# HKUST-Aerial-Robotics/MIND

Hardware: AMD Instinct MI355X
Metric: sim steps/sec (whole node) + scenario-tree nodes expanded/sec, AV2 demo scenes (higher is better)
Workload: dtype f32-class (bf16 hi+mid+lo split operands = 24 significand bits, six products, fp32 accumulate) pair kernel + ActorNet, f32 elsewhere in the predictor, f64 iLQR

## Files before the change

include/mind_hip.h:

```cpp
#ifndef MIND_HIP_H
#define MIND_HIP_H

#include <stddef.h>
#include <stdint.h>

#ifdef __cplusplus
extern "C" {
#endif

#define MIND_OK 0
#define MIND_EINVAL (-1)
#define MIND_ENOMEM (-2)
#define MIND_EHIP (-3)
#define MIND_ESTATE (-4)
#define MIND_ENOTFOUND (-5)

typedef struct mind_ctx mind_ctx;

int mind_ctx_create(int device, void *stream, mind_ctx **out);
int mind_ctx_destroy(mind_ctx *ctx);
const char *mind_last_error_string(mind_ctx *ctx);
int mind_ctx_synchronize(mind_ctx *ctx);

typedef struct {
// ... 44 lines not shown
#define MIND_PAIR_BF16X6 3
int mind_set_pair_precision(mind_ctx *ctx, int mode);

int mind_set_tuning(mind_ctx *ctx, const char *name, int value);
int mind_get_pair_precision(mind_ctx *ctx);
int mind_debug_pack_bfrag(const float *w, int row_stride, uint32_t *out);

int mind_debug_pair_schedule(const int *scene_tokens, const int *scene_actors, int n_scenes, int n_cu, int last_layer, int *out_jobs, int cap,
                             int *out_info);

int mind_debug_actor_lw_plan(int n_actors, int np, int chunk, long long *out_launches, int cap, long long *out_info);

int mind_debug_pack_conv_frag(const float *w, int co, int ci, int ksz, uint32_t *out, size_t cap);

int mind_debug_trig(mind_ctx *ctx, const double *x, int n, double *out);

int mind_debug_set_layers(mind_ctx *ctx, int n);
int64_t mind_debug_read(mind_ctx *ctx, const char *name, float *host, int64_t max_floats);

typedef struct {
  int n_nodes;
  const int32_t *parent;
  const float *prob;
  int n_agents;
  const float *agent_mean;
  const float *agent_cov;
  const double *field;
  const double *node_w;
} mind_cost_tree;

// ... 283 lines not shown
```

mind_amd/_lib.py:

```python
import ctypes as C
import os

_HERE = os.path.dirname(os.path.abspath(__file__))
LIB_PATH = os.environ.get("MIND_HIP_LIB", os.path.join(_HERE, "libmind_hip.so"))

MIND_OK = 0
MIND_EINVAL, MIND_ENOMEM, MIND_EHIP, MIND_ESTATE, MIND_ENOTFOUND = -1, -2, -3, -4, -5


class TensorDesc(C.Structure):
    _fields_ = [("name", C.c_char_p), ("data", C.POINTER(C.c_float)), ("numel", C.c_int64)]


class SceneBatch(C.Structure):
    _fields_ = [("n_scenes", C.c_int), ("actor_off", C.POINTER(C.c_int32)), ("lane_off", C.POINTER(C.c_int32)),
                ("actors", C.c_void_p), ("lanes", C.c_void_p), ("lane_feat", C.c_void_p),
                ("actor_ctrs", C.c_void_p), ("actor_vecs", C.c_void_p), ("lane_ctrs", C.c_void_p),
                ("lane_vecs", C.c_void_p), ("rpe", C.POINTER(C.c_void_p)), ("tgt_nodes", C.c_void_p),
                ("tgt_rpe", C.c_void_p)]


class PredOut(C.Structure):
    _fields_ = [("cls", C.c_void_p), ("reg", C.c_void_p), ("vel", C.c_void_p), ("lane_feat", C.c_void_p),
                ("actor_emb", C.c_void_p), ("cls_emb", C.c_void_p)]
# ... 119 lines not shown
    _fields_ = [("time_ahead", C.c_double), ("min_vel", C.c_float), ("dist_thres", C.c_float), ("max_depth", C.c_int), ("max_rounds", C.c_int),
                ("pred_len", C.c_int), ("prob_floor", C.c_float), ("cfg_warm", C.c_void_p), ("cfg_full", C.c_void_p), ("speculative", C.c_int),
                ("ego_type_slot", C.c_int)]


class PlannerOut(C.Structure):
    _fields_ = [("n_plans", C.c_longlong),
                ("n_agents", C.c_int), ("n_trees", C.c_int), ("best", C.c_int), ("n_expanded", C.c_int), ("n_rounds", C.c_int), ("n_traj_nodes", C.c_int),
                ("costs", C.POINTER(C.c_double)), ("ctrl", C.c_double * 2), ("aime_s", C.c_double), ("ilqr_s", C.c_double), ("total_s", C.c_double),
                ("tot", LoopTotals)]


EXPORTS = ["mind_ctx_create", "mind_ctx_destroy", "mind_last_error_string", "mind_ctx_synchronize",
           "mind_weights_load", "mind_predict_batch", "mind_last_fusion_stats", "mind_last_actor_stats", "mind_debug_actor_lw_plan", "mind_set_profiling",
           "mind_ilqr_solve_trees", "mind_ilqr_contingency", "mind_ilqr_solve_fields", "mind_cost_eval", "mind_lane_dist_field", "mind_aime_world", "mind_aime_rebase", "mind_debug_set_layers",
           "mind_debug_read", "mind_set_pair_precision", "mind_get_pair_precision", "mind_debug_pack_bfrag", "mind_debug_pack_conv_frag", "mind_debug_pair_schedule", "mind_set_tuning", "mind_last_ilqr_stats", "mind_aime_plan", "mind_last_ilqr_profile", "mind_eval_traj_trees", "mind_last_ilqr_trace", "mind_ilqr_contingency_begin", "mind_ilqr_finish", "mind_fill_tracks", "mind_ilqr_contingency_begin_plan", "mind_debug_trig", "mind_aime_plan_begin", "mind_aime_plan_poll", "mind_aime_plan_finish", "mind_ctx_busy", "mind_ilqr_finish_plan",
           "mind_set_exchange", "mind_last_exchange_stats",
           "mind_loop_create", "mind_loop_destroy", "mind_loop_reset", "mind_loop_advance", "mind_loop_state", "mind_loop_last_plan", "mind_loop_export",
           "mind_planner_create", "mind_planner_destroy", "mind_planner_reset", "mind_planner_observe", "mind_planner_set_lanes", "mind_planner_set_target_lane",
           "mind_planner_set_solve_lane", "mind_planner_set_eval_lane", "mind_planner_plan", "mind_planner_last_plan", "mind_planner_export"]

EXCHANGE_FN = C.CFUNCTYPE(C.c_int, C.c_void_p, C.c_int, C.c_void_p, C.c_void_p, C.c_int64)
XCHG_ALLGATHER, XCHG_ALLREDUCE, XCHG_ALLTOALLV = 0, 1, 2

_lib = None


def load():
    global _lib
    if _lib is not None:
        return _lib
# ... 41 lines not shown
    lib.mind_aime_plan_poll.argtypes = [C.c_void_p]
    lib.mind_aime_plan_finish.argtypes = [C.c_void_p, C.POINTER(AimePlanOut)]
    lib.mind_ctx_busy.argtypes = [C.c_void_p]
    lib.mind_ilqr_finish_plan.argtypes = [C.c_void_p, C.c_int, C.c_int, C.c_void_p, C.c_void_p, C.c_void_p, C.c_void_p]
    lib.mind_set_pair_precision.argtypes = [C.c_void_p, C.c_int]
    lib.mind_set_tuning.argtypes = [C.c_void_p, C.c_char_p, C.c_int]
    lib.mind_last_ilqr_stats.argtypes = [C.c_void_p, C.POINTER(C.c_float), C.POINTER(C.c_int), C.POINTER(C.c_int)]
    lib.mind_last_ilqr_profile.argtypes = [C.c_void_p, C.POINTER(C.c_double)]
    lib.mind_last_ilqr_trace.argtypes = [C.c_void_p, C.c_int, C.c_int, C.POINTER(C.c_double), C.c_int, C.POINTER(C.c_int)]
    lib.mind_eval_traj_trees.argtypes = [C.POINTER(C.c_double), C.POINTER(C.c_double), C.POINTER(C.c_int32), C.c_int, C.c_void_p, C.c_int, C.c_int,
                                         C.c_double, C.POINTER(C.c_double)]
    lib.mind_get_pair_precision.argtypes = [C.c_void_p]
    lib.mind_debug_pack_bfrag.argtypes = [C.POINTER(C.c_float), C.c_int, C.POINTER(C.c_uint32)]
    lib.mind_debug_pair_schedule.argtypes = [C.POINTER(C.c_int), C.POINTER(C.c_int), C.c_int, C.c_int, C.c_int, C.POINTER(C.c_int), C.c_int, C.POINTER(C.c_int)]
    lib.mind_debug_trig.argtypes = [C.c_void_p, C.POINTER(C.c_double), C.c_int, C.POINTER(C.c_double)]
    lib.mind_debug_pack_conv_frag.argtypes = [C.POINTER(C.c_float), C.c_int, C.c_int, C.c_int, C.POINTER(C.c_uint32), C.c_size_t]
    lib.mind_debug_set_layers.argtypes = [C.c_void_p, C.c_int]
    lib.mind_debug_read.argtypes = [C.c_void_p, C.c_char_p, C.POINTER(C.c_float), C.c_int64]
    lib.mind_set_exchange.argtypes = [C.c_void_p, C.c_int, C.c_int, EXCHANGE_FN, C.c_void_p, C.c_int]
    lib.mind_last_exchange_stats.argtypes = [C.c_void_p, C.POINTER(C.c_longlong), C.POINTER(C.c_longlong)]
    lib.mind_loop_create.argtypes = [C.c_void_p, C.POINTER(LoopDesc), C.POINTER(C.c_void_p)]
    lib.mind_loop_destroy.argtypes = [C.c_void_p]
    lib.mind_loop_reset.argtypes = [C.c_void_p]
    lib.mind_loop_advance.argtypes = [C.c_void_p, C.c_int, C.c_double, C.c_longlong, C.POINTER(LoopOut)]
    lib.mind_loop_state.argtypes = [C.c_void_p, C.POINTER(LoopOut)]
    lib.mind_loop_last_plan.argtypes = [C.c_void_p, C.POINTER(AimePlanOut)] + [C.POINTER(C.c_void_p)] * 6 + [C.c_void_p]
    lib.mind_loop_export.argtypes = [C.c_void_p, C.c_int, C.POINTER(C.c_int), C.c_void_p, C.c_void_p, C.c_void_p]
    lib.mind_planner_create.argtypes = [C.c_void_p, C.POINTER(PlannerDesc), C.POINTER(C.c_void_p)]
    lib.mind_planner_destroy.argtypes = [C.c_void_p]
    lib.mind_planner_reset.argtypes = [C.c_void_p]
# ... 26 lines not shown
```

mind_amd/csrc/actor_mfma_kernels.hip:

```cpp
#include <hip/hip_runtime.h>
#include <stdint.h>

#define AM_T 1024
#ifdef MIND_ACTOR_TRACE
__device__ long long am_tr_[64];
__device__ int am_trn_;
#define AM_MARK() do { if (blockIdx.x == 0 && threadIdx.x == 0) { const long long n_ = clock64(); am_tr_[am_trn_ & 63] = n_; ++am_trn_; } } while (0)
#else
#define AM_MARK() do {} while (0)
#endif
#define AM_WAVES 16
#define AM_MAXT 2
#define AM_RSD(C) (3 * (C) / 2 + 4)
#define AM_BUF 2496
#define AM_XIN 0
#define AM_O0 1344
#define AM_FA (AM_O0 + 7 * AM_BUF)
#define AM_RED (AM_FA + 48 * AM_RSD(128))
#define AM_LDS_DWORDS (AM_RED + 64)

struct AmRes { const u32 *c1, *c2, *ds; const float *g1, *b1, *g2, *b2, *gd, *bd; };
struct AmLat { const u32 *w; const float *g, *b; };
struct AmW {
  AmRes res[9];
  AmLat lat[4];
};
typedef u32 u32x2 __attribute__((ext_vector_type(2)));

__device__ __forceinline__ float am_block_sum(float v, float *red, int flip) {
  v = wave_sum(v);
  float *r = red + (flip & 1) * 32;
  if ((threadIdx.x & 63) == 0) r[threadIdx.x >> 6] = v;
  __syncthreads();
  float s = 0.f;
#pragma unroll
  for (int w = 0; w < AM_WAVES; ++w) s += r[w];
  return s;
}

template <int NP>
__device__ __forceinline__ void am_store_split(u32 *rowp, int plane, const f32x4 &y) {
  u32x2 h, m, l;
  h[0] = pk_bf16(y[0], y[1]); h[1] = pk_bf16(y[2], y[3]);
  *(u32x2 *)rowp = h;
  if (NP == 1) return;
  const float r0 = y[0] - bf_lo_f32(h[0]), r1 = y[1] - bf_hi_f32(h[0]), r2 = y[2] - bf_lo_f32(h[1]), r3 = y[3] - bf_hi_f32(h[1]);
  m[0] = pk_bf16(r0, r1); m[1] = pk_bf16(r2, r3);
  *(u32x2 *)(rowp + plane) = m;
  l[0] = pk_bf16(r0 - bf_lo_f32(m[0]), r1 - bf_hi_f32(m[0])); l[1] = pk_bf16(r2 - bf_lo_f32(m[1]), r3 - bf_hi_f32(m[1]));
  *(u32x2 *)(rowp + 2 * plane) = l;
}
template <int NP>
// ... 44 lines not shown
      acc[i] = MFMA_BF(ah, bh, acc[i]);
      if (NP >= 3) {
        if (NP == 6) {
          corr = MFMA_BF(al, bh, corr);
          corr = MFMA_BF(ah, bl, corr);
          corr = MFMA_BF(am, bm, corr);
        }
        corr = MFMA_BF(am, bh, corr);
        corr = MFMA_BF(ah, bm, corr);
      }
    }
    if (NP >= 3) acc[i] += corr;
  }
}

template <int NP>
__device__ __forceinline__ void am_gn(f32x4 (&acc)[AM_MAXT], int Cout, int Tout, const float *__restrict__ g,
                                      const float *__restrict__ b, const u32 *resid, const float *up, bool relu, u32 *outs,
                                      float *outf, float *__restrict__ gout, float *red) {
  const int lane = threadIdx.x & 63, wave = threadIdx.x >> 6;
  const int r = lane & 15, q = lane >> 4;
  const int ntt = (Tout + 15) >> 4;
  const int tiles = (Cout >> 4) * ntt;
  const int RSD = AM_RSD(Cout), PLANE = Cout >> 1;
  f32x4 gg[AM_MAXT], bb[AM_MAXT];
  float s = 0.f;
#pragma unroll
  for (int i = 0; i < AM_MAXT; ++i) {
    const int ti = wave + AM_WAVES * i;
    if (ti >= tiles) continue;
    const int mt = ti / ntt, nt = ti - mt * ntt;
    gg[i] = *(const f32x4 *)(g + mt * 16 + q * 4);
    bb[i] = *(const f32x4 *)(b + mt * 16 + q * 4);
    if (nt * 16 + r < Tout) s += (acc[i][0] + acc[i][1]) + (acc[i][2] + acc[i][3]);
  }
  const float n = (float)(Cout * Tout);
  const float mean = am_block_sum(s, red, 0) / n;
  float v = 0.f;
#pragma unroll
  for (int i = 0; i < AM_MAXT; ++i) {
    const int ti = wave + AM_WAVES * i;
    if (ti >= tiles) continue;
    const int nt = ti % ntt;
    if (nt * 16 + r < Tout) {
#pragma unroll
      for (int e = 0; e < 4; ++e) { const float d = acc[i][e] - mean; v = fmaf(d, d, v); }
    }
  }
  const float rstd = 1.0f / sqrtf(am_block_sum(v, red, 1) / n + 1e-5f);
#pragma unroll
  for (int i = 0; i < AM_MAXT; ++i) {
    const int ti = wave + AM_WAVES * i;
    if (ti >= tiles) continue;
    const int mt = ti / ntt, nt = ti - mt * ntt;
    const int t = nt * 16 + r, co = mt * 16 + q * 4;
    if (t >= Tout) continue;
    f32x4 y;
#pragma unroll
    for (int e = 0; e < 4; ++e) y[e] = (acc[i][e] - mean) * rstd * gg[i][e] + bb[i][e];
    if (resid) y += am_load_split<NP>(resid + t * RSD + (co >> 1), PLANE);
    if (up) {
      const int Th = Tout >> 1;
      float sp = (t + 0.5f) * 0.5f - 0.5f;
      sp = sp < 0.f ? 0.f : sp;
// ... 4 lines not shown
#pragma unroll
      for (int e = 0; e < 4; ++e) y[e] += (1.0f - l1) * a0[e] + l1 * a1[e];
    }
    if (relu) {
#pragma unroll
      for (int e = 0; e < 4; ++e) y[e] = fmaxf(y[e], 0.f);
    }
    if (gout) {
      if (t == Tout - 1) *(f32x4 *)(gout + co) = y;
    } else if (outf) {
      *(f32x4 *)(outf + t * 132 + co) = y;
    } else {
      am_store_split<NP>(outs + t * RSD + (co >> 1), PLANE, y);
    }
  }
  __syncthreads();
}

template <int NP, int LGCI, int LGCO, int STRIDE, bool DS>
__device__ __forceinline__ void am_res(const u32 *in, int Tin, const AmRes &W, u32 *out, u32 *t1, u32 *t2, float *red) {
  constexpr int Cout = 1 << LGCO;
  const int Tout = Tin / STRIDE;
  f32x4 acc[AM_MAXT];
  am_conv<NP, LGCI, 3, STRIDE>(in, Tin, W.c1, Cout, Tout, acc);
  AM_MARK();
  am_gn<NP>(acc, Cout, Tout, W.g1, W.b1, nullptr, nullptr, true, t1, nullptr, nullptr, red);
  AM_MARK();
  const u32 *resid = in;
  if (DS) {
    am_conv<NP, LGCI, 1, STRIDE>(in, Tin, W.ds, Cout, Tout, acc);
    AM_MARK();
    am_gn<NP>(acc, Cout, Tout, W.gd, W.bd, nullptr, nullptr, false, t2, nullptr, nullptr, red);
    AM_MARK();
    resid = t2;
  }
  am_conv<NP, LGCO, 3, 1>(t1, Tout, W.c2, Cout, Tout, acc);
  AM_MARK();
  am_gn<NP>(acc, Cout, Tout, W.g2, W.b2, resid, nullptr, true, out, nullptr, nullptr, red);
  AM_MARK();
}

template <int NP, int LGC>
__device__ __forceinline__ void am_lateral(const u32 *src, int T, const AmLat &W, const float *up, float *dstf, u32 *dsts,
                                           float *red) {
  f32x4 acc[AM_MAXT];
  am_conv<NP, LGC, 3, 1>(src, T, W.w, 128, T, acc);
  AM_MARK();
  am_gn<NP>(acc, 128, T, W.g, W.b, nullptr, up, false, dsts, dstf, nullptr, red);
  AM_MARK();
}

template <int NP>
__global__ __launch_bounds__(AM_T) void k_actor_mfma(const float *__restrict__ actors , int n_actors,
                                                     float *__restrict__ out , AmW W) {
  extern __shared__ __attribute__((aligned(16))) u32 smu[];
  u32 *xin = smu + AM_XIN;
  u32 *o0 = smu + AM_O0, *o1 = o0 + AM_BUF, *o2 = o1 + AM_BUF, *o3 = o2 + AM_BUF;
  u32 *ta = o3 + AM_BUF, *tb = ta + AM_BUF, *tc = tb + AM_BUF;
  u32 *fa = smu + AM_FA;
  float *red = (float *)(smu + AM_RED);
  const int tid = threadIdx.x;
  const int a = blockIdx.x;
  if (a >= n_actors) return;
  if (tid < 48 * 8) {
    const int t = tid >> 3, c = (tid & 7) * 2;
    const float v0 = c < 14 ? actors[((size_t)a * 14 + c) * 48 + t] : 0.f;
    const float v1 = c + 1 < 14 ? actors[((size_t)a * 14 + c + 1) * 48 + t] : 0.f;
    u32 *p = xin + t * AM_RSD(16) + (c >> 1);
    const u32 h = pk_bf16(v0, v1);
    const float r0 = v0 - bf_lo_f32(h), r1 = v1 - bf_hi_f32(h);
    const u32 m = pk_bf16(r0, r1);
    p[0] = h; p[8] = m; p[16] = pk_bf16(r0 - bf_lo_f32(m), r1 - bf_hi_f32(m));
  }
  __syncthreads();
#ifdef MIND_ACTOR_TRACE
  if (blockIdx.x == 0 && tid == 0) am_trn_ = 0;
#endif
  AM_MARK();
  am_res<NP, 4, 5, 1, true>(xin, 48, W.res[0], ta, tb, tc, red);
  am_res<NP, 5, 5, 1, false>(ta, 48, W.res[1], o0, tb, tc, red);
  am_res<NP, 5, 6, 2, true>(o0, 48, W.res[2], ta, tb, tc, red);
  am_res<NP, 6, 6, 1, false>(ta, 24, W.res[3], o1, tb, tc, red);
  am_res<NP, 6, 7, 2, true>(o1, 24, W.res[4], ta, tb, tc, red);
  am_res<NP, 7, 7, 1, false>(ta, 12, W.res[5], o2, tb, tc, red);
  am_res<NP, 7, 8, 2, true>(o2, 12, W.res[6], ta, tb, tc, red);
  am_res<NP, 8, 8, 1, false>(ta, 6, W.res[7], o3, tb, tc, red);
  am_lateral<NP, 8>(o3, 6, W.lat[3], nullptr, (float *)ta, nullptr, red);
  am_lateral<NP, 7>(o2, 12, W.lat[2], (const float *)ta, (float *)tb, nullptr, red);
  am_lateral<NP, 6>(o1, 24, W.lat[1], (const float *)tb, (float *)o2, nullptr, red);
  am_lateral<NP, 5>(o0, 48, W.lat[0], (const float *)o2, nullptr, fa, red);
  {
    const AmRes &R = W.res[8];
    f32x4 acc[AM_MAXT];
    am_conv<NP, 7, 3, 1>(fa, 48, R.c1, 128, 48, acc);
    AM_MARK();
    am_gn<NP>(acc, 128, 48, R.g1, R.b1, nullptr, nullptr, true, o0, nullptr, nullptr, red);
    AM_MARK();
    am_conv<NP, 7, 3, 1>(o0, 48, R.c2, 128, 48, acc);
    AM_MARK();
    am_gn<NP>(acc, 128, 48, R.g2, R.b2, fa, nullptr, true, nullptr, nullptr, out + (size_t)a * 128, red);
    AM_MARK();
  }
#ifdef MIND_ACTOR_TRACE
  if (blockIdx.x == 0 && tid == 0) {
    printf("[k_actor_mfma<%d>] cycles conv/gn per stage:", NP);
    for (int q = 1; q < am_trn_ && q < 64; ++q) printf(" %lld", am_tr_[q] - am_tr_[q - 1]);
    printf("\n");
  }
#endif
}
extern "C" size_t mind_actor_mfma_lds_bytes() { return (size_t)AM_LDS_DWORDS * sizeof(u32); }
```

mind_amd/csrc/encdec_kernels.hip:

```cpp
#include <hip/hip_runtime.h>
#include <stdint.h>

typedef float f32x4 __attribute__((ext_vector_type(4)));

#define NT 256

__device__ __forceinline__ float wave_sum(float v) {
  v += __shfl_xor(v, 32, 64);
  v += __shfl_xor(v, 16, 64);
  v += __shfl_xor(v, 8, 64);
  v += __shfl_xor(v, 4, 64);
  v += __shfl_xor(v, 2, 64);
  v += __shfl_xor(v, 1, 64);
  return v;
}

__device__ __forceinline__ float block_sum(float v, float *red) {
  v = wave_sum(v);
  __syncthreads();
  if ((threadIdx.x & 63) == 0) red[threadIdx.x >> 6] = v;
  __syncthreads();
  return red[0] + red[1] + red[2] + red[3];
}

#ifndef DB
#define DB 16
#endif
#define DENSE_ROW_FENCE() __builtin_amdgcn_sched_barrier(0)
#define DBQ 8
template <int R>
__device__ __forceinline__ void dense_quads(const float *in, int ldi, int K, const float *__restrict__ WT,
                                            const float *__restrict__ b, int NOUT, float *out, int ldo,
                                            float *part, int part_floats) {
  const int nthr = blockDim.x;
  const int NQ = NOUT >> 2;
  int KP = 1;
  while (KP * 2 * NQ <= nthr && KP * 2 * R * NOUT <= part_floats && KP * 2 <= (K >> 2)) KP *= 2;
// ... 940 lines not shown
```

mind_amd/csrc/fusion_kernels.hip:

```cpp
#include <hip/hip_runtime.h>
#include <stdint.h>

typedef float f32x4 __attribute__((ext_vector_type(4)));
typedef float f32x16 __attribute__((ext_vector_type(16)));

typedef unsigned int u32;
typedef u32 u32x4 __attribute__((ext_vector_type(4)));
typedef __bf16 bf16x8 __attribute__((ext_vector_type(8)));
typedef __bf16 bf16x2_t __attribute__((ext_vector_type(2)));
typedef float f32x2_t __attribute__((ext_vector_type(2)));

__device__ __forceinline__ u32 pk_bf16(float a, float b) {
  f32x2_t v = {a, b};
  return __builtin_bit_cast(u32, __builtin_convertvector(v, bf16x2_t));
}
__device__ __forceinline__ float bf_lo_f32(u32 pk) { return __builtin_bit_cast(float, pk << 16); }
__device__ __forceinline__ float bf_hi_f32(u32 pk) { return __builtin_bit_cast(float, pk & 0xffff0000u); }

#define D_ 128
#define PART_STRIDE 1040

struct PairJob {
  long long edge_base;
  int N;
// ... 21 lines not shown
#define LDS_WAE 0
#define LDS_WAP 16384
#define LDS_STAGE 32768
#define LDS_PTAB (LDS_STAGE + PAIR_WAVES * STAGE_FLOATS)
#define LDS_SVEC (LDS_PTAB + PAIR_WAVES * 128)
#define LDS_VT (LDS_SVEC + PAIR_WAVES * 136)
#define LDS_RT (LDS_VT + VT_SIZE)
#define LDS_TOTAL (LDS_RT + 1024)

#define LDS_FENCE() asm volatile("s_waitcnt lgkmcnt(0)" ::: "memory")
#define SCHED_FENCE() __builtin_amdgcn_sched_barrier(0)
#define OPAQUE(x) asm volatile("" : "+v"(x))

typedef f32x4 frag8[8];

__device__ __forceinline__ float red_quad(float v) {
  v += __shfl_xor(v, 16, 64);
  v += __shfl_xor(v, 32, 64);
  return v;
}
__device__ __forceinline__ float red_max16(float v) {
  v = fmaxf(v, __shfl_xor(v, 8, 64));
  v = fmaxf(v, __shfl_xor(v, 4, 64));
  v = fmaxf(v, __shfl_xor(v, 2, 64));
  v = fmaxf(v, __shfl_xor(v, 1, 64));
  return v;
}
__device__ __forceinline__ float red_sum16(float v) {
  v += __shfl_xor(v, 8, 64);
  v += __shfl_xor(v, 4, 64);
  v += __shfl_xor(v, 2, 64);
  v += __shfl_xor(v, 1, 64);
  return v;
}

__device__ __forceinline__ void ln_pairs(frag8 &a, const float *vtq, int off_g, int off_b, bool relu) {
  float s = 0.f;
#pragma unroll
  for (int b = 0; b < 8; ++b)
#pragma unroll
    for (int w = 0; w < 4; ++w) s += a[b][w];
  s = red_quad(s);
  const float mean = s * (1.0f / 128.0f);
  float v = 0.f;
#pragma unroll
  for (int b = 0; b < 8; ++b)
#pragma unroll
    for (int w = 0; w < 4; ++w) {
      const float d = a[b][w] - mean;
// ... 459 lines not shown
__device__ __forceinline__ void ksum(const float (&acc)[TP], float bias, float *rk, int kg, int col, float &r0, float &r1) {
  constexpr int TPW = TP;
  __syncthreads();
#pragma unroll
  for (int t = 0; t < TPW; ++t) rk[(kg * TPW + t) * 128 + col] = acc[t];
  __syncthreads();
  const int t0 = (TP / TKG) * kg;
  r0 = ((rk[(0 * TPW + t0) * 128 + col] + rk[(1 * TPW + t0) * 128 + col]) +
        (rk[(2 * TPW + t0) * 128 + col] + rk[(3 * TPW + t0) * 128 + col])) + bias;
  r1 = 0.f;
  if (TP / TKG == 2)
    r1 = ((rk[(0 * TPW + t0 + 1) * 128 + col] + rk[(1 * TPW + t0 + 1) * 128 + col]) +
          (rk[(2 * TPW + t0 + 1) * 128 + col] + rk[(3 * TPW + t0 + 1) * 128 + col])) + bias;
}

__device__ __forceinline__ void gsum2(float &a, float &b, float *rd, int kg, int tid) {
#pragma unroll
  for (int o = 32; o > 0; o >>= 1) { a += __shfl_xor(a, o, 64); b += __shfl_xor(b, o, 64); }
  const int wv = (tid >> 6) & 1;
  __syncthreads();
  if ((tid & 63) == 0) { rd[(kg * 2 + wv) * 2] = a; rd[(kg * 2 + wv) * 2 + 1] = b; }
  __syncthreads();
  a = rd[(kg * 2) * 2] + rd[(kg * 2 + 1) * 2];
  b = rd[(kg * 2) * 2 + 1] + rd[(kg * 2 + 1) * 2 + 1];
}

__device__ __forceinline__ void ln2tok(float &p0, float &p1, float g, float be, float *rd, int kg, int tid) {
  float s0 = p0, s1 = p1;
  gsum2(s0, s1, rd, kg, tid);
  const float d0 = p0 - s0 * (1.0f / 128.0f), d1 = p1 - s1 * (1.0f / 128.0f);
  s0 = d0 * d0; s1 = d1 * d1;
  gsum2(s0, s1, rd, kg, tid);
  p0 = d0 * (1.0f / sqrtf(s0 * (1.0f / 128.0f) + 1e-5f)) * g + be;
  p1 = d1 * (1.0f / sqrtf(s1 * (1.0f / 128.0f) + 1e-5f)) * g + be;
}

template <int TPW, bool MG>
__device__ __forceinline__ void k_token_body(const TokMeta *__restrict__ meta, int n_tok, int mode,
                                             const float *__restrict__ actor_feat,
                                             const float *__restrict__ lane_feat, float *__restrict__ x,
                                             const float *__restrict__ part, float *__restrict__ ST,
                                             float *__restrict__ QK, const TokWeights &W) {
  __shared__ __attribute__((aligned(16))) float xs[TPW][132];
  __shared__ __attribute__((aligned(16))) float tmp[TPW][260];
  __shared__ __attribute__((aligned(16))) float mb[TPW][8][132];
  __shared__ float rk[(MG ? 3 : 1) * TKG * TPW * 128];
  __shared__ float rd[TKG * 2 * 2];
  __shared__ float cw[TPW][8][8];
  const int tid = threadIdx.x, kg = tid >> 7, col = tid & 127;
  const int tok0 = blockIdx.x * TPW;
  const int nt = min(TPW, n_tok - tok0);
  constexpr bool TWO = TPW / TKG == 2;
  const int ta = (TPW / TKG) * kg, tb = TWO ? ta + 1 : ta;
  const bool va = ta < nt, vb = TWO && tb < nt;
#ifdef MIND_TOKEN_TRACE
  long long tt_[10] = {0, 0, 0, 0, 0, 0, 0, 0, 0, 0}, tq_ = clock64();
#define TT(i) do { const long long n_ = clock64(); tt_[i] += n_ - tq_; tq_ = n_; } while (0)
#else
#define TT(i) do {} while (0)
#endif

  if (mode & 1) {
// ... 9 lines not shown
      const TokMeta m = meta[tok0 + tb];
      tyb = m.type;
      if (m.type == 0) fb = actor_feat[(size_t)m.src * 128 + col];
      else if (m.type == 1) fb = lane_feat[(size_t)m.src * 128 + col];
    }
    tmp[ta][col] = fa; if (TWO) tmp[tb][col] = fb;
    __syncthreads();
    float acc[TPW], a0, a1, l0, l1;
    matvec_part<128, TPW>(acc, W.WpaT, 128, col, &tmp[0][0], 260, kg);
    ksum<TPW>(acc, W.bpa[col], rk, kg, col, a0, a1);
    matvec_part<128, TPW>(acc, W.WplT, 128, col, &tmp[0][0], 260, kg);
    ksum<TPW>(acc, W.bpl[col], rk, kg, col, l0, l1);
    float p0 = tya == 0 ? a0 : l0, p1 = tyb == 0 ? a1 : l1;
    {
      float s0 = p0, s1 = p1;
      gsum2(s0, s1, rd, kg, tid);
      const float d0 = p0 - s0 * (1.0f / 128.0f), d1 = p1 - s1 * (1.0f / 128.0f);
      s0 = d0 * d0; s1 = d1 * d1;
      gsum2(s0, s1, rd, kg, tid);
      const float ga = W.gpa[col], gl = W.gpl[col], ba = W.bepa[col], bl = W.bepl[col];
      p0 = fmaxf(d0 * (1.0f / sqrtf(s0 * (1.0f / 128.0f) + 1e-5f)) * (tya == 0 ? ga : gl) + (tya == 0 ? ba : bl), 0.f);
      p1 = fmaxf(d1 * (1.0f / sqrtf(s1 * (1.0f / 128.0f) + 1e-5f)) * (tyb == 0 ? ga : gl) + (tyb == 0 ? ba : bl), 0.f);
      if (tya == 2) p0 = 0.f;
      if (tyb == 2) p1 = 0.f;
    }
    xs[ta][col] = p0; if (TWO) xs[tb][col] = p1;
    __syncthreads();
  } else {
    xs[ta][col] = va ? x[(size_t)(tok0 + ta) * 128 + col] : 0.f;
    if (TWO) xs[tb][col] = vb ? x[(size_t)(tok0 + tb) * 128 + col] : 0.f;
    __syncthreads();
  }
  TT(0);
  if (mode & 2) {
// ... 207 lines not shown
```

mind_amd/csrc/mind_hip.hip:

```cpp
#include <hip/hip_runtime.h>

#include <cmath>
#include <cstdarg>
#include <cstdio>
#include <cstdlib>
#include <algorithm>
#include <cstring>
#include <map>
#include <string>
#include <thread>
#include <atomic>
#include <functional>
#include <vector>

#include "../../include/mind_hip.h"
#include "encdec_kernels.hip"
#include "fusion_kernels.hip"
#include "pair_bf16_kernels.hip"
#include "pair_tile_kernels.hip"
#include "pair_tile6_kernels.hip"
#include "token_mfma_kernels.hip"
#include "actor_mfma_kernels.hip"
#include "actor_lw_kernels.hip"
#include "actor_f32_kernels.hip"
// ... 2449 lines not shown
  if (!c || !x || !out || n <= 0) return MIND_EINVAL;
  HIPCHK(c, hipSetDevice(c->device));
  double *d = nullptr;
  HIPCHK(c, hipMalloc((void **)&d, (size_t)n * 5 * sizeof(double)));
  hipError_t e = hipMemcpy(d, x, (size_t)n * sizeof(double), hipMemcpyHostToDevice);
  if (e == hipSuccess) {
    hipLaunchKernelGGL(k_debug_trig, dim3((n + 63) / 64), dim3(64), 0, c->stream, d, n, d + n);
    e = hipStreamSynchronize(c->stream);
  }
  if (e == hipSuccess) e = hipMemcpy(out, d + n, (size_t)n * 4 * sizeof(double), hipMemcpyDeviceToHost);
  (void)hipFree(d);
  if (e != hipSuccess) return fail(c, MIND_EHIP, "mind_debug_trig: %s", hipGetErrorString(e));
  return MIND_OK;
}

extern "C" int mind_debug_set_layers(mind_ctx *c, int n) {
  if (!c || n < 0 || n > 6) return MIND_EINVAL;
  c->debug_layers = n;
  return MIND_OK;
}
extern "C" int64_t mind_debug_read(mind_ctx *c, const char *name, float *host, int64_t max_floats) {
  if (!c || !name) return MIND_EINVAL;
  const void *src = nullptr;
  int64_t n = 0;
  std::string k = name;
  if (k == "x") { src = c->x.p; n = (int64_t)c->last_ntok * 128; }
  else if (k == "ST") { src = c->ST.p; n = (int64_t)c->last_ntok * 256; }
  else if (k == "QK") { src = c->QK.p; n = (int64_t)c->last_ntok * 1024; }
  else if (k == "edge") { src = c->edge.p; n = c->last_edge_pairs * 128; }
  else if (k == "part") { src = c->part.p; n = (int64_t)c->last_slots * PART_STRIDE; }
// ... 57 lines not shown
```

mind_amd/csrc/token_mfma_kernels.hip:

```cpp
#define TM_TOK 16
#define TM_THREADS 256
#define TM_LDX 132
#define TM_LDT 260
#define TM_HP 8

struct TokWeightsM {
  const float *Wv, *Wo, *W1a, *W1b, *W2a, *W2b;
  const float *Ws, *Wt, *Wq, *Wkf;
  const float *Wpa, *Wpl;
};

typedef float tm_f4 __attribute__((ext_vector_type(4)));

struct TmFrag { tm_f4 a0[8], a1[8]; };
__device__ __forceinline__ void tm_load(TmFrag &F, const float *__restrict__ Wf, int ob0, int lane) {
  const tm_f4 *A = reinterpret_cast<const tm_f4 *>(Wf) + (size_t)ob0 * 8 * 64 + lane;
#pragma unroll
  for (int s4 = 0; s4 < 8; ++s4) { F.a0[s4] = A[s4 * 64]; F.a1[s4] = A[(8 + s4) * 64]; }
}
template <int BF>
__device__ __forceinline__ void tm_mma(tm_f4 (&acc)[2], const TmFrag &F, int ob0, const float *xb, int ob_stride, int lane) {
  if (BF) {
    const float *b0p = xb + 8 * (lane >> 4) + (size_t)ob0 * ob_stride;
    const float *b1p = b0p + ob_stride;
// ... 40 lines not shown
template <int BF>
__device__ __forceinline__ void tm_gemm(tm_f4 (&acc)[2], const float *__restrict__ Wf, int ob0, const float *xb, int ob_stride, int lane) {
  TmFrag F;
  tm_load(F, Wf, ob0, lane);
  tm_mma<BF>(acc, F, ob0, xb, ob_stride, lane);
}

#define TM_FEAT(ob, i) (16 * (ob) + 4 * (lane >> 4) + (i))

__device__ __forceinline__ void tm_layernorm(float *tile, int ld, const float *__restrict__ g, const float *__restrict__ be, bool relu, int tid) {
  const int row = tid >> 4, part = tid & 15;
  float *p = tile + row * ld + part * 8;
  float v[8], s = 0.f;
#pragma unroll
  for (int k = 0; k < 8; ++k) { v[k] = p[k]; s += v[k]; }
#pragma unroll
  for (int o = 8; o > 0; o >>= 1) s += __shfl_xor(s, o, 64);
  const float mean = s * (1.0f / 128.0f);
  float q = 0.f;
#pragma unroll
  for (int k = 0; k < 8; ++k) { v[k] -= mean; q += v[k] * v[k]; }
#pragma unroll
  for (int o = 8; o > 0; o >>= 1) q += __shfl_xor(q, o, 64);
  const float inv = 1.0f / sqrtf(q * (1.0f / 128.0f) + 1e-5f);
#pragma unroll
  for (int k = 0; k < 8; ++k) {
    float y = v[k] * inv * g[part * 8 + k] + be[part * 8 + k];
    p[k] = relu ? fmaxf(y, 0.f) : y;
  }
}

template <int BF>
__global__ __launch_bounds__(TM_THREADS) void k_token_mfma(const TokMeta *__restrict__ meta, int n_tok, int mode, const float *__restrict__ actor_feat,
                                                           const float *__restrict__ lane_feat, float *__restrict__ x, const float *__restrict__ part,
                                                           float *__restrict__ ST, float *__restrict__ QK, TokWeights W, TokWeightsM WM) {
  extern __shared__ __attribute__((aligned(16))) float tm_sm[];
  float *xs = tm_sm;
  float *tmp = xs + TM_TOK * TM_LDX;
// ... 229 lines not shown
```

Before: 1789.

## Use DPP/permlane cross-lane reductions, fuse GN pairs, and split conv tiles

Adds a shared cross-lane header that replaces __shfl_xor reductions with DPP row moves and permlane16/32 swaps. Block reductions now alternate between two scratch buffers, which removes the leading barrier. In the actor net, the downsample conv is computed before the first group norm so both group norms share one pair of block reductions. The 128x48 convs now use a variant that spreads the MFMA tiles over all waves and exchanges them through LDS. A debug entry point for checking the reductions is also added, and the change uses more LDS and registers.

```diff
diff --git a/include/mind_hip.h b/include/mind_hip.h
--- a/include/mind_hip.h
+++ b/include/mind_hip.h
@@ -82,6 +82,7 @@
 int mind_debug_pack_conv_frag(const float *w, int co, int ci, int ksz, uint32_t *out, size_t cap);
 
 int mind_debug_trig(mind_ctx *ctx, const double *x, int n, double *out);
+int mind_debug_xlane(mind_ctx *ctx, const float *in, int rows, int kind, float *out);
 
 int mind_debug_set_layers(mind_ctx *ctx, int n);
 int64_t mind_debug_read(mind_ctx *ctx, const char *name, float *host, int64_t max_floats);
diff --git a/mind_amd/_lib.py b/mind_amd/_lib.py
--- a/mind_amd/_lib.py
+++ b/mind_amd/_lib.py
@@ -157,7 +157,7 @@
 EXPORTS = ["mind_ctx_create", "mind_ctx_destroy", "mind_last_error_string", "mind_ctx_synchronize",
            "mind_weights_load", "mind_predict_batch", "mind_last_fusion_stats", "mind_last_actor_stats", "mind_debug_actor_lw_plan", "mind_set_profiling",
            "mind_ilqr_solve_trees", "mind_ilqr_contingency", "mind_ilqr_solve_fields", "mind_cost_eval", "mind_lane_dist_field", "mind_aime_world", "mind_aime_rebase", "mind_debug_set_layers",
-           "mind_debug_read", "mind_set_pair_precision", "mind_get_pair_precision", "mind_debug_pack_bfrag", "mind_debug_pack_conv_frag", "mind_debug_pair_schedule", "mind_set_tuning", "mind_last_ilqr_stats", "mind_aime_plan", "mind_last_ilqr_profile", "mind_eval_traj_trees", "mind_last_ilqr_trace", "mind_ilqr_contingency_begin", "mind_ilqr_finish", "mind_fill_tracks", "mind_ilqr_contingency_begin_plan", "mind_debug_trig", "mind_aime_plan_begin", "mind_aime_plan_poll", "mind_aime_plan_finish", "mind_ctx_busy", "mind_ilqr_finish_plan",
+           "mind_debug_read", "mind_set_pair_precision", "mind_get_pair_precision", "mind_debug_pack_bfrag", "mind_debug_pack_conv_frag", "mind_debug_pair_schedule", "mind_set_tuning", "mind_last_ilqr_stats", "mind_aime_plan", "mind_last_ilqr_profile", "mind_eval_traj_trees", "mind_last_ilqr_trace", "mind_ilqr_contingency_begin", "mind_ilqr_finish", "mind_fill_tracks", "mind_ilqr_contingency_begin_plan", "mind_debug_trig", "mind_debug_xlane", "mind_aime_plan_begin", "mind_aime_plan_poll", "mind_aime_plan_finish", "mind_ctx_busy", "mind_ilqr_finish_plan",
            "mind_set_exchange", "mind_last_exchange_stats",
            "mind_loop_create", "mind_loop_destroy", "mind_loop_reset", "mind_loop_advance", "mind_loop_state", "mind_loop_last_plan", "mind_loop_export",
            "mind_planner_create", "mind_planner_destroy", "mind_planner_reset", "mind_planner_observe", "mind_planner_set_lanes", "mind_planner_set_target_lane",
@@ -229,6 +229,7 @@
     lib.mind_debug_pack_bfrag.argtypes = [C.POINTER(C.c_float), C.c_int, C.POINTER(C.c_uint32)]
     lib.mind_debug_pair_schedule.argtypes = [C.POINTER(C.c_int), C.POINTER(C.c_int), C.c_int, C.c_int, C.c_int, C.POINTER(C.c_int), C.c_int, C.POINTER(C.c_int)]
     lib.mind_debug_trig.argtypes = [C.c_void_p, C.POINTER(C.c_double), C.c_int, C.POINTER(C.c_double)]
+    lib.mind_debug_xlane.argtypes = [C.c_void_p, C.POINTER(C.c_float), C.c_int, C.c_int, C.POINTER(C.c_float)]
     lib.mind_debug_pack_conv_frag.argtypes = [C.POINTER(C.c_float), C.c_int, C.c_int, C.c_int, C.POINTER(C.c_uint32), C.c_size_t]
     lib.mind_debug_set_layers.argtypes = [C.c_void_p, C.c_int]
     lib.mind_debug_read.argtypes = [C.c_void_p, C.c_char_p, C.POINTER(C.c_float), C.c_int64]
diff --git a/mind_amd/csrc/actor_mfma_kernels.hip b/mind_amd/csrc/actor_mfma_kernels.hip
--- a/mind_amd/csrc/actor_mfma_kernels.hip
+++ b/mind_amd/csrc/actor_mfma_kernels.hip
@@ -17,7 +17,8 @@
 #define AM_O0 1344
 #define AM_FA (AM_O0 + 7 * AM_BUF)
 #define AM_RED (AM_FA + 48 * AM_RSD(128))
-#define AM_LDS_DWORDS (AM_RED + 64)
+#define AM_XF (AM_RED + 64)
+#define AM_LDS_DWORDS (AM_XF + 24 * 64 * 4)
 
 struct AmRes { const u32 *c1, *c2, *ds; const float *g1, *b1, *g2, *b2, *gd, *bd; };
 struct AmLat { const u32 *w; const float *g, *b; };
@@ -36,6 +37,17 @@
 #pragma unroll
   for (int w = 0; w < AM_WAVES; ++w) s += r[w];
   return s;
+}
+
+__device__ __forceinline__ void am_block_sum2(float &a, float &b, float *red, int flip) {
+  wave_sum2(a, b);
+  float *r = red + (flip & 1) * 32;
+  if ((threadIdx.x & 63) == 0) { r[threadIdx.x >> 6] = a; r[16 + (threadIdx.x >> 6)] = b; }
+  __syncthreads();
+  float sa = 0.f, sb = 0.f;
+#pragma unroll
+  for (int w = 0; w < AM_WAVES; ++w) { sa += r[w]; sb += r[16 + w]; }
+  a = sa; b = sb;
 }
 
 template <int NP>
@@ -110,16 +122,65 @@
   }
 }
 
-template <int NP>
-__device__ __forceinline__ void am_gn(f32x4 (&acc)[AM_MAXT], int Cout, int Tout, const float *__restrict__ g,
-                                      const float *__restrict__ b, const u32 *resid, const float *up, bool relu, u32 *outs,
-                                      float *outf, float *__restrict__ gout, float *red) {
+template <int NP, int LGC, int KSZ, int STRIDE>
+__device__ __forceinline__ void am_conv_mt2(const u32 *in, int Tin, const u32 *__restrict__ Wf, int Tout, f32x4 (&acc)[AM_MAXT],
+                                            f32x4 *xf) {
+  static_assert(AM_MAXT == 2, "two tiles per wave");
+  constexpr int CP = 1 << LGC, RSD = AM_RSD(CP), PLANE = CP / 2, PAD = (KSZ - 1) / 2;
+  constexpr int KS = (KSZ * CP + 31) / 32;
   const int lane = threadIdx.x & 63, wave = threadIdx.x >> 6;
   const int r = lane & 15, q = lane >> 4;
-  const int ntt = (Tout + 15) >> 4;
-  const int tiles = (Cout >> 4) * ntt;
-  const int RSD = AM_RSD(Cout), PLANE = Cout >> 1;
-  f32x4 gg[AM_MAXT], bb[AM_MAXT];
+  const int mt = wave & 7, nt0 = wave < 8 ? 0 : 2;
+  const bool two = wave < 8;
+  const u32 *wp = Wf + (size_t)mt * KS * 768 + lane * 4;
+  f32x4 a2[2], corr[2];
+#pragma unroll
+  for (int j = 0; j < 2; ++j) { a2[j] = (f32x4){0.f, 0.f, 0.f, 0.f}; corr[j] = (f32x4){0.f, 0.f, 0.f, 0.f}; }
+#pragma unroll 2
+  for (int ks = 0; ks < KS; ++ks) {
+    const u32x4 ah = *(const u32x4 *)(wp + (size_t)ks * 768);
+    u32x4 am, al;
+    if (NP >= 3) am = *(const u32x4 *)(wp + (size_t)ks * 768 + 256);
+    if (NP == 6) al = *(const u32x4 *)(wp + (size_t)ks * 768 + 512);
+    const int k0 = ks * 32 + q * 8;
+    const int dk = k0 >> LGC, ci = k0 & (CP - 1);
+#pragma unroll
+    for (int j = 0; j < 2; ++j) {
+      if (j == 1 && !two) continue;
+      const int t = (nt0 + j) * 16 + r;
+      const int row = t * STRIDE + dk - PAD;
+      u32x4 bh = {0u, 0u, 0u, 0u}, bm = {0u, 0u, 0u, 0u}, bl = {0u, 0u, 0u, 0u};
+      if (dk < KSZ && t < Tout && row >= 0 && row < Tin) {
+        const u32 *bp = in + row * RSD + (ci >> 1);
+        bh = *(const u32x4 *)bp;
+        if (NP >= 3) bm = *(const u32x4 *)(bp + PLANE);
+        if (NP == 6) bl = *(const u32x4 *)(bp + 2 * PLANE);
+      }
+      a2[j] = MFMA_BF(ah, bh, a2[j]);
+      if (NP >= 3) {
+        if (NP == 6) {
+          corr[j] = MFMA_BF(al, bh, corr[j]);
+          corr[j] = MFMA_BF(ah, bl, corr[j]);
+          corr[j] = MFMA_BF(am, bm, corr[j]);
+        }
+        corr[j] = MFMA_BF(am, bh, corr[j]);
+        corr[j] = MFMA_BF(ah, bm, corr[j]);
+      }
+    }
+  }
+  if (NP >= 3) { a2[0] += corr[0]; a2[1] += corr[1]; }
+  xf[(mt * 3 + nt0) * 64 + lane] = a2[0];
+  if (two) xf[(mt * 3 + 1) * 64 + lane] = a2[1];
+  __syncthreads();
+  acc[0] = xf[wave * 64 + lane];
+  acc[1] = (f32x4){0.f, 0.f, 0.f, 0.f};
+  if (wave < 8) acc[1] = xf[(wave + AM_WAVES) * 64 + lane];
+}
+
+__device__ __forceinline__ float am_gn_sum(const f32x4 (&acc)[AM_MAXT], int tiles, int ntt, int Tout, const float *__restrict__ g,
+                                           const float *__restrict__ b, f32x4 (&gg)[AM_MAXT], f32x4 (&bb)[AM_MAXT]) {
+  const int lane = threadIdx.x & 63, wave = threadIdx.x >> 6;
+  const int r = lane & 15, q = lane >> 4;
   float s = 0.f;
 #pragma unroll
   for (int i = 0; i < AM_MAXT; ++i) {
@@ -130,8 +191,11 @@
     bb[i] = *(const f32x4 *)(b + mt * 16 + q * 4);
     if (nt * 16 + r < Tout) s += (acc[i][0] + acc[i][1]) + (acc[i][2] + acc[i][3]);
   }
-  const float n = (float)(Cout * Tout);
-  const float mean = am_block_sum(s, red, 0) / n;
+  return s;
+}
+__device__ __forceinline__ float am_gn_dev(const f32x4 (&acc)[AM_MAXT], int tiles, int ntt, int Tout, float mean) {
+  const int lane = threadIdx.x & 63, wave = threadIdx.x >> 6;
+  const int r = lane & 15;
   float v = 0.f;
 #pragma unroll
   for (int i = 0; i < AM_MAXT; ++i) {
@@ -143,7 +207,17 @@
       for (int e = 0; e < 4; ++e) { const float d = acc[i][e] - mean; v = fmaf(d, d, v); }
     }
   }
-  const float rstd = 1.0f / sqrtf(am_block_sum(v, red, 1) / n + 1e-5f);
+  return v;
+}
+template <int NP>
+__device__ __forceinline__ void am_gn_out(const f32x4 (&acc)[AM_MAXT], int Cout, int Tout, float mean, float rstd,
+                                          const f32x4 (&gg)[AM_MAXT], const f32x4 (&bb)[AM_MAXT], const u32 *resid, const float *up,
+                                          bool relu, u32 *outs, float *outf, float *__restrict__ gout) {
+  const int lane = threadIdx.x & 63, wave = threadIdx.x >> 6;
+  const int r = lane & 15, q = lane >> 4;
+  const int ntt = (Tout + 15) >> 4;
+  const int tiles = (Cout >> 4) * ntt;
+  const int RSD = AM_RSD(Cout), PLANE = Cout >> 1;
 #pragma unroll
   for (int i = 0; i < AM_MAXT; ++i) {
     const int ti = wave + AM_WAVES * i;
@@ -178,6 +252,42 @@
       am_store_split<NP>(outs + t * RSD + (co >> 1), PLANE, y);
     }
   }
+}
+
+template <int NP>
+__device__ __forceinline__ void am_gn(f32x4 (&acc)[AM_MAXT], int Cout, int Tout, const float *__restrict__ g,
+                                      const float *__restrict__ b, const u32 *resid, const float *up, bool relu, u32 *outs,
+                                      float *outf, float *__restrict__ gout, float *red) {
+  const int ntt = (Tout + 15) >> 4;
+  const int tiles = (Cout >> 4) * ntt;
+  f32x4 gg[AM_MAXT], bb[AM_MAXT];
+  const float s = am_gn_sum(acc, tiles, ntt, Tout, g, b, gg, bb);
+  const float n = (float)(Cout * Tout);
+  const float mean = am_block_sum(s, red, 0) / n;
+  const float v = am_gn_dev(acc, tiles, ntt, Tout, mean);
+  const float rstd = 1.0f / sqrtf(am_block_sum(v, red, 1) / n + 1e-5f);
+  am_gn_out<NP>(acc, Cout, Tout, mean, rstd, gg, bb, resid, up, relu, outs, outf, gout);
+  __syncthreads();
+}
+
+template <int NP>
+__device__ __forceinline__ void am_gn2(f32x4 (&a)[AM_MAXT], f32x4 (&d)[AM_MAXT], int Cout, int Tout, const float *__restrict__ ga,
+                                       const float *__restrict__ ba, u32 *outa, const float *__restrict__ gd,
+                                       const float *__restrict__ bd, u32 *outd, float *red) {
+  const int ntt = (Tout + 15) >> 4;
+  const int tiles = (Cout >> 4) * ntt;
+  f32x4 gga[AM_MAXT], bba[AM_MAXT], ggd[AM_MAXT], bbd[AM_MAXT];
+  float sa = am_gn_sum(a, tiles, ntt, Tout, ga, ba, gga, bba);
+  float sd = am_gn_sum(d, tiles, ntt, Tout, gd, bd, ggd, bbd);
+  const float n = (float)(Cout * Tout);
+  am_block_sum2(sa, sd, red, 0);
+  const float mean_a = sa / n, mean_d = sd / n;
+  float va = am_gn_dev(a, tiles, ntt, Tout, mean_a);
+  float vd = am_gn_dev(d, tiles, ntt, Tout, mean_d);
+  am_block_sum2(va, vd, red, 1);
+  const float rstd_a = 1.0f / sqrtf(va / n + 1e-5f), rstd_d = 1.0f / sqrtf(vd / n + 1e-5f);
+  am_gn_out<NP>(a, Cout, Tout, mean_a, rstd_a, gga, bba, nullptr, nullptr, true, outa, nullptr, nullptr);
+  am_gn_out<NP>(d, Cout, Tout, mean_d, rstd_d, ggd, bbd, nullptr, nullptr, false, outd, nullptr, nullptr);
   __syncthreads();
 }
 
@@ -188,15 +298,17 @@
   f32x4 acc[AM_MAXT];
   am_conv<NP, LGCI, 3, STRIDE>(in, Tin, W.c1, Cout, Tout, acc);
   AM_MARK();
-  am_gn<NP>(acc, Cout, Tout, W.g1, W.b1, nullptr, nullptr, true, t1, nullptr, nullptr, red);
-  AM_MARK();
   const u32 *resid = in;
   if (DS) {
-    am_conv<NP, LGCI, 1, STRIDE>(in, Tin, W.ds, Cout, Tout, acc);
-    AM_MARK();
-    am_gn<NP>(acc, Cout, Tout, W.gd, W.bd, nullptr, nullptr, false, t2, nullptr, nullptr, red);
+    f32x4 accd[AM_MAXT];
+    am_conv<NP, LGCI, 1, STRIDE>(in, Tin, W.ds, Cout, Tout, accd);
+    AM_MARK();
+    am_gn2<NP>(acc, accd, Cout, Tout, W.g1, W.b1, t1, W.gd, W.bd, t2, red);
     AM_MARK();
     resid = t2;
+  } else {
+    am_gn<NP>(acc, Cout, Tout, W.g1, W.b1, nullptr, nullptr, true, t1, nullptr, nullptr, red);
+    AM_MARK();
   }
   am_conv<NP, LGCO, 3, 1>(t1, Tout, W.c2, Cout, Tout, acc);
   AM_MARK();
@@ -204,11 +316,12 @@
   AM_MARK();
 }
 
-template <int NP, int LGC>
+template <int NP, int LGC, bool MT2 = false >
 __device__ __forceinline__ void am_lateral(const u32 *src, int T, const AmLat &W, const float *up, float *dstf, u32 *dsts,
-                                           float *red) {
+                                           float *red, f32x4 *xf = nullptr) {
   f32x4 acc[AM_MAXT];
-  am_conv<NP, LGC, 3, 1>(src, T, W.w, 128, T, acc);
+  if (MT2) am_conv_mt2<NP, LGC, 3, 1>(src, T, W.w, T, acc, xf);
+  else am_conv<NP, LGC, 3, 1>(src, T, W.w, 128, T, acc);
   AM_MARK();
   am_gn<NP>(acc, 128, T, W.g, W.b, nullptr, up, false, dsts, dstf, nullptr, red);
   AM_MARK();
@@ -223,6 +336,7 @@
   u32 *ta = o3 + AM_BUF, *tb = ta + AM_BUF, *tc = tb + AM_BUF;
   u32 *fa = smu + AM_FA;
   float *red = (float *)(smu + AM_RED);
+  f32x4 *xf = (f32x4 *)(smu + AM_XF);
   const int tid = threadIdx.x;
   const int a = blockIdx.x;
   if (a >= n_actors) return;
@@ -252,15 +366,15 @@
   am_lateral<NP, 8>(o3, 6, W.lat[3], nullptr, (float *)ta, nullptr, red);
   am_lateral<NP, 7>(o2, 12, W.lat[2], (const float *)ta, (float *)tb, nullptr, red);
   am_lateral<NP, 6>(o1, 24, W.lat[1], (const float *)tb, (float *)o2, nullptr, red);
-  am_lateral<NP, 5>(o0, 48, W.lat[0], (const float *)o2, nullptr, fa, red);
+  am_lateral<NP, 5, true>(o0, 48, W.lat[0], (const float *)o2, nullptr, fa, red, xf);
   {
     const AmRes &R = W.res[8];
     f32x4 acc[AM_MAXT];
-    am_conv<NP, 7, 3, 1>(fa, 48, R.c1, 128, 48, acc);
+    am_conv_mt2<NP, 7, 3, 1>(fa, 48, R.c1, 48, acc, xf);
     AM_MARK();
     am_gn<NP>(acc, 128, 48, R.g1, R.b1, nullptr, nullptr, true, o0, nullptr, nullptr, red);
     AM_MARK();
-    am_conv<NP, 7, 3, 1>(o0, 48, R.c2, 128, 48, acc);
+    am_conv_mt2<NP, 7, 3, 1>(o0, 48, R.c2, 48, acc, xf);
     AM_MARK();
     am_gn<NP>(acc, 128, 48, R.g2, R.b2, fa, nullptr, true, nullptr, nullptr, out + (size_t)a * 128, red);
     AM_MARK();
diff --git a/mind_amd/csrc/encdec_kernels.hip b/mind_amd/csrc/encdec_kernels.hip
--- a/mind_amd/csrc/encdec_kernels.hip
+++ b/mind_amd/csrc/encdec_kernels.hip
@@ -1,26 +1,17 @@
 #include <hip/hip_runtime.h>
 #include <stdint.h>
+#include "mind_xlane.h"
 
 typedef float f32x4 __attribute__((ext_vector_type(4)));
 
 #define NT 256
 
-__device__ __forceinline__ float wave_sum(float v) {
-  v += __shfl_xor(v, 32, 64);
-  v += __shfl_xor(v, 16, 64);
-  v += __shfl_xor(v, 8, 64);
-  v += __shfl_xor(v, 4, 64);
-  v += __shfl_xor(v, 2, 64);
-  v += __shfl_xor(v, 1, 64);
-  return v;
-}
-
-__device__ __forceinline__ float block_sum(float v, float *red) {
+__device__ __forceinline__ float block_sum(float v, float *red, int flip) {
   v = wave_sum(v);
-  __syncthreads();
-  if ((threadIdx.x & 63) == 0) red[threadIdx.x >> 6] = v;
-  __syncthreads();
-  return red[0] + red[1] + red[2] + red[3];
+  float *r = red + (flip & 1) * 4;
+  if ((threadIdx.x & 63) == 0) r[threadIdx.x >> 6] = v;
+  __syncthreads();
+  return r[0] + r[1] + r[2] + r[3];
 }
 
 #ifndef DB
diff --git a/mind_amd/csrc/fusion_kernels.hip b/mind_amd/csrc/fusion_kernels.hip
--- a/mind_amd/csrc/fusion_kernels.hip
+++ b/mind_amd/csrc/fusion_kernels.hip
@@ -1,5 +1,6 @@
 #include <hip/hip_runtime.h>
 #include <stdint.h>
+#include "mind_xlane.h"
 
 typedef float f32x4 __attribute__((ext_vector_type(4)));
 typedef float f32x16 __attribute__((ext_vector_type(16)));
@@ -59,25 +60,9 @@
 
 typedef f32x4 frag8[8];
 
-__device__ __forceinline__ float red_quad(float v) {
-  v += __shfl_xor(v, 16, 64);
-  v += __shfl_xor(v, 32, 64);
-  return v;
-}
-__device__ __forceinline__ float red_max16(float v) {
-  v = fmaxf(v, __shfl_xor(v, 8, 64));
-  v = fmaxf(v, __shfl_xor(v, 4, 64));
-  v = fmaxf(v, __shfl_xor(v, 2, 64));
-  v = fmaxf(v, __shfl_xor(v, 1, 64));
-  return v;
-}
-__device__ __forceinline__ float red_sum16(float v) {
-  v += __shfl_xor(v, 8, 64);
-  v += __shfl_xor(v, 4, 64);
-  v += __shfl_xor(v, 2, 64);
-  v += __shfl_xor(v, 1, 64);
-  return v;
-}
+__device__ __forceinline__ float red_quad(float v) { return xl_quad_sum(v); }
+__device__ __forceinline__ float red_max16(float v) { return xl_row_max(v); }
+__device__ __forceinline__ float red_sum16(float v) { return xl_row_sum(v); }
 
 __device__ __forceinline__ void ln_pairs(frag8 &a, const float *vtq, int off_g, int off_b, bool relu) {
   float s = 0.f;
@@ -567,23 +552,22 @@
           (rk[(2 * TPW + t0 + 1) * 128 + col] + rk[(3 * TPW + t0 + 1) * 128 + col])) + bias;
 }
 
-__device__ __forceinline__ void gsum2(float &a, float &b, float *rd, int kg, int tid) {
-#pragma unroll
-  for (int o = 32; o > 0; o >>= 1) { a += __shfl_xor(a, o, 64); b += __shfl_xor(b, o, 64); }
+__device__ __forceinline__ void gsum2(float &a, float &b, float *rd, int kg, int tid, int flip) {
+  wave_sum2(a, b);
   const int wv = (tid >> 6) & 1;
+  float *r = rd + (flip & 1) * (TKG * 2 * 2);
+  if ((tid & 63) == 0) { r[(kg * 2 + wv) * 2] = a; r[(kg * 2 + wv) * 2 + 1] = b; }
   __syncthreads();
-  if ((tid & 63) == 0) { rd[(kg * 2 + wv) * 2] = a; rd[(kg * 2 + wv) * 2 + 1] = b; }
-  __syncthreads();
-  a = rd[(kg * 2) * 2] + rd[(kg * 2 + 1) * 2];
-  b = rd[(kg * 2) * 2 + 1] + rd[(kg * 2 + 1) * 2 + 1];
+  a = r[(kg * 2) * 2] + r[(kg * 2 + 1) * 2];
+  b = r[(kg * 2) * 2 + 1] + r[(kg * 2 + 1) * 2 + 1];
 }
 
 __device__ __forceinline__ void ln2tok(float &p0, float &p1, float g, float be, float *rd, int kg, int tid) {
   float s0 = p0, s1 = p1;
-  gsum2(s0, s1, rd, kg, tid);
+  gsum2(s0, s1, rd, kg, tid, 0);
   const float d0 = p0 - s0 * (1.0f / 128.0f), d1 = p1 - s1 * (1.0f / 128.0f);
   s0 = d0 * d0; s1 = d1 * d1;
-  gsum2(s0, s1, rd, kg, tid);
+  gsum2(s0, s1, rd, kg, tid, 1);
   p0 = d0 * (1.0f / sqrtf(s0 * (1.0f / 128.0f) + 1e-5f)) * g + be;
   p1 = d1 * (1.0f / sqrtf(s1 * (1.0f / 128.0f) + 1e-5f)) * g + be;
 }
@@ -598,7 +582,7 @@
   __shared__ __attribute__((aligned(16))) float tmp[TPW][260];
   __shared__ __attribute__((aligned(16))) float mb[TPW][8][132];
   __shared__ float rk[(MG ? 3 : 1) * TKG * TPW * 128];
-  __shared__ float rd[TKG * 2 * 2];
+  __shared__ float rd[2 * TKG * 2 * 2];
   __shared__ float cw[TPW][8][8];
   const int tid = threadIdx.x, kg = tid >> 7, col = tid & 127;
   const int tok0 = blockIdx.x * TPW;
@@ -638,10 +622,10 @@
     float p0 = tya == 0 ? a0 : l0, p1 = tyb == 0 ? a1 : l1;
     {
       float s0 = p0, s1 = p1;
-      gsum2(s0, s1, rd, kg, tid);
+      gsum2(s0, s1, rd, kg, tid, 0);
       const float d0 = p0 - s0 * (1.0f / 128.0f), d1 = p1 - s1 * (1.0f / 128.0f);
       s0 = d0 * d0; s1 = d1 * d1;
-      gsum2(s0, s1, rd, kg, tid);
+      gsum2(s0, s1, rd, kg, tid, 1);
       const float ga = W.gpa[col], gl = W.gpl[col], ba = W.bepa[col], bl = W.bepl[col];
       p0 = fmaxf(d0 * (1.0f / sqrtf(s0 * (1.0f / 128.0f) + 1e-5f)) * (tya == 0 ? ga : gl) + (tya == 0 ? ba : bl), 0.f);
       p1 = fmaxf(d1 * (1.0f / sqrtf(s1 * (1.0f / 128.0f) + 1e-5f)) * (tyb == 0 ? ga : gl) + (tyb == 0 ? ba : bl), 0.f);
diff --git a/mind_amd/csrc/mind_hip.hip b/mind_amd/csrc/mind_hip.hip
--- a/mind_amd/csrc/mind_hip.hip
+++ b/mind_amd/csrc/mind_hip.hip
@@ -2487,6 +2487,49 @@
   return MIND_OK;
 }
 
+__global__ __launch_bounds__(1024) void k_debug_xlane(const float *__restrict__ in, int kind, float *__restrict__ out) {
+  __shared__ float red[64];
+  const int tid = threadIdx.x, lane = tid & 63;
+  const size_t row0 = (size_t)blockIdx.x * (blockDim.x >> 6), row = row0 + (tid >> 6);
+  const float v = in[row * 64 + lane];
+  if (kind == 0) out[row * 64 + lane] = wave_sum(v);
+  else if (kind == 1) out[row * 64 + lane] = xl_row_sum(v);
+  else if (kind == 2) out[row * 64 + lane] = xl_row_max(v);
+  else if (kind == 3) {
+    const int kg = tid >> 7;
+    const float w = in[(row0 + 7 - (tid >> 6)) * 64 + lane];
+    float a = v, b = w;
+    gsum2(a, b, red, kg, tid, 0);
+    float c = w, d = v;
+    gsum2(c, d, red, kg, tid, 1);
+    float *o = out + (row * 64 + lane) * 4;
+    o[0] = a; o[1] = b; o[2] = c; o[3] = d;
+  } else {
+    float *o = out + row * 192 + lane;
+    o[0] = am_block_sum(v, red, 0);
+    o[64] = am_block_sum(in[row * 64 + 63 - lane], red, 1);
+    o[128] = am_block_sum(-v, red, 0);
+  }
+}
+extern "C" int mind_debug_xlane(mind_ctx *c, const float *in, int rows, int kind, float *out) {
+  if (!c || !in || !out || rows <= 0 || kind < 0 || kind > 4) return MIND_EINVAL;
+  const int rpb = kind == 3 ? 8 : kind == 4 ? 16 : 4, per = kind == 3 ? 256 : kind == 4 ? 192 : 64;
+  if (rows % rpb) return fail(c, MIND_EINVAL, "mind_debug_xlane: kind %d needs a multiple of %d rows", kind, rpb);
+  HIPCHK(c, hipSetDevice(c->device));
+  float *d = nullptr;
+  const size_t n_in = (size_t)rows * 64, n_out = (size_t)rows * per;
+  HIPCHK(c, hipMalloc((void **)&d, (n_in + n_out) * sizeof(float)));
+  hipError_t e = hipMemcpy(d, in, n_in * sizeof(float), hipMemcpyHostToDevice);
+  if (e == hipSuccess) {
+    hipLaunchKernelGGL(k_debug_xlane, dim3(rows / rpb), dim3(64 * rpb), 0, c->stream, d, kind, d + n_in);
+    e = hipStreamSynchronize(c->stream);
+  }
+  if (e == hipSuccess) e = hipMemcpy(out, d + n_in, n_out * sizeof(float), hipMemcpyDeviceToHost);
+  (void)hipFree(d);
+  if (e != hipSuccess) return fail(c, MIND_EHIP, "mind_debug_xlane: %s", hipGetErrorString(e));
+  return MIND_OK;
+}
+
 extern "C" int mind_debug_set_layers(mind_ctx *c, int n) {
   if (!c || n < 0 || n > 6) return MIND_EINVAL;
   c->debug_layers = n;
diff --git a/mind_amd/csrc/mind_xlane.h b/mind_amd/csrc/mind_xlane.h
--- /dev/null
+++ b/mind_amd/csrc/mind_xlane.h
@@ -0,0 +1,75 @@
+#pragma once
+#include <hip/hip_runtime.h>
+
+namespace xl_detail {
+typedef unsigned u2 __attribute__((ext_vector_type(2)));
+struct Add { static __device__ __forceinline__ float op(float a, float b) { return a + b; } };
+struct Max { static __device__ __forceinline__ float op(float a, float b) { return fmaxf(a, b); } };
+
+template <int CTRL, int BANK_MASK>
+__device__ __forceinline__ int dpp(int old, int v) {
+  return __builtin_amdgcn_update_dpp(old, v, CTRL, 0xf, BANK_MASK, BANK_MASK == 0xf);
+}
+template <int OFF>
+__device__ __forceinline__ float partner(float v) {
+  static_assert(OFF == 8 || OFF == 4 || OFF == 2 || OFF == 1, "row offsets are 8, 4, 2, 1");
+  const int x = __float_as_int(v);
+  if (OFF == 8) return __int_as_float(dpp<0x128, 0xf>(x, x));
+  if (OFF == 4) return __int_as_float(dpp<0x114, 0xa>(dpp<0x104, 0x5>(x, x), x));
+  if (OFF == 2) return __int_as_float(dpp<0x4e, 0xf>(x, x));
+  return __int_as_float(dpp<0xb1, 0xf>(x, x));
+}
+template <class OP, int OFF>
+__device__ __forceinline__ float step(float v) {
+  static_assert(OFF == 32 || OFF == 16 || OFF == 8 || OFF == 4 || OFF == 2 || OFF == 1, "offset must be a power of two below 64");
+  if (OFF == 32) {
+    const u2 r = __builtin_amdgcn_permlane32_swap(__float_as_uint(v), __float_as_uint(v), false, false);
+    return OP::op(__uint_as_float(r[0]), __uint_as_float(r[1]));
+  }
+  if (OFF == 16) {
+    const u2 r = __builtin_amdgcn_permlane16_swap(__float_as_uint(v), __float_as_uint(v), false, false);
+    return OP::op(__uint_as_float(r[0]), __uint_as_float(r[1]));
+  }
+  return OP::op(v, partner<(OFF < 16 ? OFF : 1)>(v));
+}
+}
+
+template <int OFF> __device__ __forceinline__ float xl_xor_add(float v) { return xl_detail::step<xl_detail::Add, OFF>(v); }
+template <int OFF> __device__ __forceinline__ float xl_xor_max(float v) { return xl_detail::step<xl_detail::Max, OFF>(v); }
+
+__device__ __forceinline__ float wave_sum(float v) {
+  v = xl_xor_add<32>(v);
+  v = xl_xor_add<16>(v);
+  v = xl_xor_add<8>(v);
+  v = xl_xor_add<4>(v);
+  v = xl_xor_add<2>(v);
+  v = xl_xor_add<1>(v);
+  return v;
+}
+__device__ __forceinline__ void wave_sum2(float &a, float &b) {
+  a = xl_xor_add<32>(a); b = xl_xor_add<32>(b);
+  a = xl_xor_add<16>(a); b = xl_xor_add<16>(b);
+  a = xl_xor_add<8>(a); b = xl_xor_add<8>(b);
+  a = xl_xor_add<4>(a); b = xl_xor_add<4>(b);
+  a = xl_xor_add<2>(a); b = xl_xor_add<2>(b);
+  a = xl_xor_add<1>(a); b = xl_xor_add<1>(b);
+}
+__device__ __forceinline__ float xl_row_sum(float v) {
+  v = xl_xor_add<8>(v);
+  v = xl_xor_add<4>(v);
+  v = xl_xor_add<2>(v);
+  v = xl_xor_add<1>(v);
+  return v;
+}
+__device__ __forceinline__ float xl_row_max(float v) {
+  v = xl_xor_max<8>(v);
+  v = xl_xor_max<4>(v);
+  v = xl_xor_max<2>(v);
+  v = xl_xor_max<1>(v);
+  return v;
+}
+__device__ __forceinline__ float xl_quad_sum(float v) {
+  v = xl_xor_add<16>(v);
+  v = xl_xor_add<32>(v);
+  return v;
+}
diff --git a/mind_amd/csrc/token_mfma_kernels.hip b/mind_amd/csrc/token_mfma_kernels.hip
--- a/mind_amd/csrc/token_mfma_kernels.hip
+++ b/mind_amd/csrc/token_mfma_kernels.hip
@@ -78,14 +78,12 @@
   float v[8], s = 0.f;
 #pragma unroll
   for (int k = 0; k < 8; ++k) { v[k] = p[k]; s += v[k]; }
-#pragma unroll
-  for (int o = 8; o > 0; o >>= 1) s += __shfl_xor(s, o, 64);
+  s = xl_row_sum(s);
   const float mean = s * (1.0f / 128.0f);
   float q = 0.f;
 #pragma unroll
   for (int k = 0; k < 8; ++k) { v[k] -= mean; q += v[k] * v[k]; }
-#pragma unroll
-  for (int o = 8; o > 0; o >>= 1) q += __shfl_xor(q, o, 64);
+  q = xl_row_sum(q);
   const float inv = 1.0f / sqrtf(q * (1.0f / 128.0f) + 1e-5f);
 #pragma unroll
   for (int k = 0; k < 8; ++k) {
```

New measurement: 1560. -12.8%, worse.
